# IntuitionMachines/volta

Measured on AMD Instinct MI355X. Metric: image-text pairs/sec, ctrl_vilbert_base pretrain step, higher is better.
Workload: dtype bf16

## Files before the change

### include/volta_hip.h

```cpp
#ifndef VOLTA_HIP_H
#define VOLTA_HIP_H
#include <stddef.h>
#include <stdint.h>

#ifdef __cplusplus
extern "C" {
#endif

typedef void* vk_stream_t;

int vk_version(void);
const char* vk_device_arch(void);
const char* vk_last_error(void);

typedef struct vk_dropout {
    const uint64_t* seed;
    uint32_t site;
    uint32_t threshold;
    float scale;
} vk_dropout;

int vk_set_seed(uint64_t* seed_dev, uint64_t seed, vk_stream_t s);

int vk_cast_f32_bf16(const float* src, void* dst, int64_t n, vk_stream_t s);
// ... 84 lines not shown

typedef struct vk_ln_bwd_args {
    const void* dy;
    const void* z;
    const float* mean;
    const float* rstd;
    const float* gamma;
    void* dz;
    void* dd;
    float* partial;
    float* dgamma;
    float* dbeta;
    const int32_t* dyn;
    int32_t M, H;
    int32_t split_row;
    int32_t post;
    float out_scale;
    int32_t accumulate;
    vk_dropout drop;
    vk_drop_rows seg[2];
} vk_ln_bwd_args;
int vk_ln_bwd_partial_rows(int M);
int vk_ln_bwd(const vk_ln_bwd_args* a, vk_stream_t s);
int vk_ln_bwd_pair(const vk_ln_bwd_args* a, const vk_ln_bwd_args* b, vk_stream_t s);
int vk_ln_bwd_finalize(const vk_ln_bwd_args* a, vk_stream_t s);

typedef struct vk_attn_args {
    const void* q[2];
    const void* k[2];
    const void* v[2];
    int32_t ld[2];
    int32_t L[2];
    const float* mask[2];
    void* ctx[2];
    int32_t ldo[2];
    float* lse[2];
    int32_t B, nh;
    int32_t gate[2][2];
    vk_dropout drop[2][2];
    float scale;
    int32_t dh;
    float* probs[2][2];
} vk_attn_args;
typedef struct vk_attn_bwd_args {
    const void* dctx[2];
    void* dq[2];
    void* dk[2];
    void* dv[2];
    int32_t ldg[2];
} vk_attn_bwd_args;
int vk_gated_attn_fwd(const vk_attn_args* a, vk_stream_t s);
int vk_gated_attn_bwd(const vk_attn_args* a, const vk_attn_bwd_args* b, vk_stream_t s);
size_t vk_gated_attn_lds_bytes(const vk_attn_args* a, int backward);

typedef struct vk_embed_args {
    const int64_t* ids;
    const int64_t* type_ids;
    const int64_t* pos_ids;
    const float* word;
    const float* pos;
    const float* type;
    const void* extra;
    void* z;
    int32_t M, T, H;
    int32_t V, P, n_types;
} vk_embed_args;
int vk_embed_sum_fwd(const vk_embed_args* a, vk_stream_t s);
typedef struct vk_embed_bwd_args {
    const void* dz;
    const int64_t* ids;
    const int64_t* type_ids;
    const int64_t* pos_ids;
    float* dword;
    float* dpos;
    float* dtype;
    int32_t M, T, H, n_types;
    int32_t V, P;
    void* work;
} vk_embed_bwd_args;
int64_t vk_embed_bwd_workspace_bytes(int M, int H, int V, int P, int has_pos);
int vk_embed_sum_bwd(const vk_embed_bwd_args* a, vk_stream_t s);

int vk_rows32(int M);
int vk_loc_linear_fwd(const float* loc, const float* W, const float* bias, void* out, int M, int H, int nloc, vk_stream_t s);
int vk_loc_linear_bwd(const void* dz, const float* loc, float* partial, float* dW, float* db, int M, int H, int nloc, vk_stream_t s);
int vk_add_dropout(const void* a, const void* b, void* y, int M, int H, float scale, vk_dropout drop, int backward, vk_stream_t s);
int vk_colsum_bf16(const void* src, float* partial, float* out, int M, int H, int accumulate, vk_stream_t s);
int vk_vlbert_prep_fwd(const float* loc, int nloc, const float* feat, const float* mask_emb, void* out, int32_t* zero_flag,
                       int M, int F, int dim, vk_dropout drop, vk_stream_t s);
int vk_vlbert_maskgrad(const void* dx, int ldx, int col0, const int32_t* zero_flag, float* partial, float* out, int M, int F,
                       vk_dropout drop, vk_stream_t s);
int vk_rowgroup_sum_bf16(const void* in, void* out, int B, int T, int H, vk_stream_t s);
int vk_relu_bwd_bf16(const void* dy, const void* y, void* out, int64_t n, vk_stream_t s);
int vk_copy_async(void* dst, const void* src, int64_t bytes, vk_stream_t s);
typedef struct vk_grad_seed_args {
    const float* src;
    int64_t stride_b, stride_l;
    void* dst;
    const void* y;
    int32_t B, L, H, row0, ld, ldy, accumulate, reserved_;
} vk_grad_seed_args;
int vk_grad_seed(const vk_grad_seed_args* a, vk_stream_t s);
#define VK_PAIR_MAX_SEGS 8
typedef struct vk_pair_gather_args {
    const void* src[VK_PAIR_MAX_SEGS];
    void* dst[VK_PAIR_MAX_SEGS];
// ... 539 lines not shown
```

### volta_amd/_lib.py

```python
import ctypes as C
import os

import torch

_HERE = os.path.dirname(os.path.abspath(__file__))
LIB_PATH = os.path.join(_HERE, "libvolta_hip_%s.so" % os.environ["VK_LIB"] if os.environ.get("VK_LIB") else "libvolta_hip.so")
GEMM_PERSISTENT, GEMM_ONE_TILE_PER_WG, GEMM_SOFT_START = 0x1000, 0x2000, 0x4000


class VoltaHipError(RuntimeError):
    pass


if not os.path.exists(LIB_PATH):
    raise ImportError(
        "volta_amd: %s not found. The HIP kernels are the product; there is no fallback path. "
        "Build with `make -C volta_amd/csrc` (hipcc --offload-arch=gfx950)." % LIB_PATH)

lib = C.CDLL(LIB_PATH)

c_p = C.c_void_p
i32 = C.c_int32
CHUNK_SKIP = 255

# ... 251 lines not shown
    _fields_ = [("fn", i32), ("p", c_p * 6), ("n", C.c_int64 * 6), ("f", C.c_float * 2), ("drop", Dropout)]


class Op(C.Structure):
    _fields_ = [("kind", i32), ("i0", i32), ("i1", i32), ("i2", i32), ("a", c_p), ("b", c_p), ("c", c_p)]


(OP_GEMM, OP_LN_FWD, OP_LN_BWD, OP_ATTN_FWD, OP_ATTN_BWD, OP_EMBED_FWD, OP_EMBED_BWD, OP_XENT_FWD, OP_XENT_BWD,
 OP_KL_FWD, OP_KL_BWD, OP_GENERIC, OP_SIDE_BEGIN, OP_SIDE_END, OP_WAIT_SIDE, OP_JOIN, OP_LN_FINALIZE, OP_GEMM_FP8, OP_GEMM_CHAIN) = range(1, 20)
(FN_CAST, FN_MEMSET, FN_LOC_FWD, FN_LOC_BWD, FN_ADD_DROPOUT, FN_COLSUM, FN_SELECT, FN_GATHER, FN_SCATTER_ADD,
 FN_LOSS_FINAL, FN_POOL_FWD, FN_POOL_BWD, FN_MASK_PREP, FN_MUL, FN_VLBERT_PREP, FN_VLBERT_MASKGRAD, FN_ROWGROUP_SUM,
 FN_RELU_BWD, FN_COPY, FN_SUM_SLABS, FN_SUM_SLABS_BF16, FN_SIDE_TAIL, FN_QUANT_ROWS, FN_CAST_FP8, FN_VIS_LOSS_FWD, FN_VIS_LOSS_BWD,
 FN_NCE_NEG, FN_TEXT_END_ROWS, FN_VLBERT_OBJ_IDS, FN_VLBERT_POSITIONS, FN_HOLD, FN_GATE, FN_BUMP, FN_GRAD_SEED, FN_LORA_FWD, FN_LORA_BWD,
 FN_LORA_PROJ_FWD, FN_LORA_PROJ_BWD, FN_LORA_FWD_DROP, FN_LORA_BWD_DROP, FN_LORA_PROJ_FWD_DROP, FN_LORA_PROJ_BWD_DROP) = range(1, 43)


class AttnArgs(C.Structure):
    _fields_ = [("q", c_p * 2), ("k", c_p * 2), ("v", c_p * 2), ("ld", i32 * 2), ("L", i32 * 2), ("mask", c_p * 2),
                ("ctx", c_p * 2), ("ldo", i32 * 2), ("lse", c_p * 2), ("B", i32), ("nh", i32), ("gate", (i32 * 2) * 2),
                ("drop", (Dropout * 2) * 2), ("scale", C.c_float), ("dh", i32), ("probs", (c_p * 2) * 2)]


class AttnBwdArgs(C.Structure):
    _fields_ = [("dctx", c_p * 2), ("dq", c_p * 2), ("dk", c_p * 2), ("dv", c_p * 2), ("ldg", i32 * 2)]


NT, NN, TN = 0, 1, 2
EPI_BF16, EPI_GELU, EPI_MULR, EPI_ADDR, EPI_F32, EPI_RELU, EPI_F32_ACC = range(7)


def _sig(name, restype, *argtypes):
    f = getattr(lib, name)
    f.restype = restype
    f.argtypes = list(argtypes)
    return f


_sig("vk_version", C.c_int)
_sig("vk_device_arch", C.c_char_p)
_sig("vk_last_error", C.c_char_p)
_sig("vk_set_seed", C.c_int, c_p, C.c_uint64, c_p)
_sig("vk_cast_f32_bf16", C.c_int, c_p, c_p, C.c_int64, c_p)
_sig("vk_gemm_grouped", C.c_int, C.c_int, C.c_int, C.POINTER(GemmProblem), C.c_int, c_p)
_sig("vk_gemm_fp8_grouped", C.c_int, C.c_int, C.POINTER(GemmFp8Problem), C.c_int, C.c_int, c_p)
_sig("vk_quant_rows_fp8", C.c_int, c_p, C.c_int, C.c_int64, c_p, C.c_int64, c_p, C.c_int, C.c_int, c_p, c_p)
_sig("vk_cast_bf16_fp8", C.c_int, c_p, c_p, C.c_int64, C.c_float, c_p)
_sig("vk_gemm_grouped_ex", C.c_int, C.c_int, C.c_int, C.POINTER(GemmProblem), C.c_int, C.c_int, c_p)
_sig("vk_gemm_geometry", C.c_int, C.c_int, C.c_int, C.POINTER(GemmProblem), C.c_int)
_sig("vk_gemm_chain", C.c_int, C.c_int, C.c_int, C.POINTER(GemmProblem), C.c_int, C.c_int, C.POINTER(GemmProblem), C.c_int, c_p)
_sig("vk_gemm_split_workspace_bytes", C.c_size_t, C.c_int, C.c_int, C.c_int, C.c_int, C.c_int, C.POINTER(C.c_int))
_sig("vk_gated_attn_fwd", C.c_int, C.POINTER(AttnArgs), c_p)
_sig("vk_gated_attn_bwd", C.c_int, C.POINTER(AttnArgs), C.POINTER(AttnBwdArgs), c_p)
_sig("vk_gated_attn_lds_bytes", C.c_size_t, C.POINTER(AttnArgs), C.c_int)
_sig("vk_ln_fwd", C.c_int, C.POINTER(LnArgs), c_p)
_sig("vk_ln_bwd_partial_rows", C.c_int, C.c_int)
_sig("vk_ln_bwd", C.c_int, C.POINTER(LnBwdArgs), c_p)
_sig("vk_embed_sum_fwd", C.c_int, C.POINTER(EmbedArgs), c_p)
_sig("vk_embed_sum_bwd", C.c_int, C.POINTER(EmbedBwdArgs), c_p)
_sig("vk_embed_bwd_workspace_bytes", C.c_int64, C.c_int, C.c_int, C.c_int, C.c_int, C.c_int)
_sig("vk_rows32", C.c_int, C.c_int)
_sig("vk_loc_linear_fwd", C.c_int, c_p, c_p, c_p, c_p, C.c_int, C.c_int, C.c_int, c_p)
_sig("vk_loc_linear_bwd", C.c_int, c_p, c_p, c_p, c_p, c_p, C.c_int, C.c_int, C.c_int, c_p)
_sig("vk_add_dropout", C.c_int, c_p, c_p, c_p, C.c_int, C.c_int, C.c_float, Dropout, C.c_int, c_p)
_sig("vk_colsum_bf16", C.c_int, c_p, c_p, c_p, C.c_int, C.c_int, C.c_int, c_p)
_sig("vk_vlbert_prep_fwd", C.c_int, c_p, C.c_int, c_p, c_p, c_p, c_p, C.c_int, C.c_int, C.c_int, Dropout, c_p)
_sig("vk_vlbert_maskgrad", C.c_int, c_p, C.c_int, C.c_int, c_p, c_p, c_p, C.c_int, C.c_int, Dropout, c_p)
_sig("vk_rowgroup_sum_bf16", C.c_int, c_p, c_p, C.c_int, C.c_int, C.c_int, c_p)
_sig("vk_relu_bwd_bf16", C.c_int, c_p, c_p, c_p, C.c_int64, c_p)
_sig("vk_copy_async", C.c_int, c_p, c_p, C.c_int64, c_p)
_sig("vk_select_rows", C.c_int, c_p, C.c_int, C.c_int, C.c_int, C.c_int, C.c_int, c_p, c_p, c_p, c_p)
_sig("vk_gather_rows", C.c_int, c_p, c_p, c_p, c_p, C.c_int, C.c_int, c_p)
_sig("vk_scatter_rows_add", C.c_int, c_p, c_p, c_p, c_p, C.c_int, C.c_int, c_p)
_sig("vk_xent_fwd", C.c_int, C.POINTER(XentArgs), c_p)
_sig("vk_xent_bwd", C.c_int, C.POINTER(XentArgs), c_p, C.c_int, c_p, c_p)
_sig("vk_kl_fwd", C.c_int, C.POINTER(KlArgs), c_p)
_sig("vk_kl_bwd", C.c_int, C.POINTER(KlArgs), c_p, C.c_int, c_p, c_p)
_sig("vk_loss_finalize", C.c_int, c_p, c_p, c_p, C.c_int, C.c_float, c_p, c_p)
_sig("vk_pool_mul_fwd", C.c_int, c_p, c_p, c_p, C.c_int, C.c_int, Dropout, c_p)
_sig("vk_pool_fuse_fwd", C.c_int, c_p, c_p, c_p, C.c_int, C.c_int, C.c_int, Dropout, c_p)
_sig("vk_pool_fuse_bwd", C.c_int, c_p, C.c_int, c_p, c_p, c_p, c_p, C.c_int, C.c_int, C.c_int, Dropout, c_p)
_sig("vk_text_end_rows", C.c_int, c_p, C.c_int, C.c_int, c_p, c_p, c_p)
_sig("vk_vlbert_obj_ids", C.c_int, c_p, c_p, C.c_int, C.c_int, c_p)
_sig("vk_lmdb_open", C.c_int, C.c_char_p, C.POINTER(c_p))
_sig("vk_lmdb_close", None, c_p)
_sig("vk_lmdb_entries", C.c_int64, c_p)
_sig("vk_lmdb_first", C.c_int, c_p)
_sig("vk_lmdb_next", C.c_int, c_p, C.POINTER(c_p), C.POINTER(C.c_size_t), C.POINTER(c_p), C.POINTER(C.c_size_t))
_sig("vk_lmdb_get", C.c_int, c_p, C.c_char_p, C.c_size_t, C.POINTER(c_p), C.POINTER(C.c_size_t))
_sig("vk_concap_record_decode", C.c_int, c_p, C.c_size_t, C.POINTER(ConcapRecord))
_sig("vk_concap_records_decode", C.c_int, C.POINTER(c_p), C.POINTER(C.c_size_t), C.POINTER(ConcapRecord), C.c_int, C.c_int, C.POINTER(C.c_int))
_sig("vk_wordpiece_open", C.c_int, C.c_char_p, C.c_int, C.POINTER(c_p))
_sig("vk_wordpiece_close", None, c_p)
_sig("vk_wordpiece_vocab_size", C.c_int, c_p)
_sig("vk_wordpiece_token_id", C.c_int, c_p, C.c_char_p)
_sig("vk_wordpiece_encode", C.c_int, c_p, C.c_char_p, C.c_size_t, c_p, C.c_int)
_sig("vk_wordpiece_encode_batch", C.c_int, c_p, C.POINTER(C.c_char_p), C.POINTER(C.c_size_t), C.c_int, c_p, C.c_int, c_p, C.c_int)
_sig("vk_b64_decode", C.c_int, C.c_char_p, C.c_size_t, c_p, C.c_size_t, C.POINTER(C.c_size_t))
_sig("vk_task_batch", C.c_int, C.POINTER(TaskBatchArgs), c_p)
_sig("vk_task_images_stage", C.c_int, C.POINTER(TaskImage), C.c_int, C.c_int, C.POINTER(C.c_int))
_sig("vk_task_batch_pool", C.c_int, C.POINTER(TaskPoolArgs), c_p)
_sig("vk_task_pool_means", C.c_int, C.POINTER(TaskPoolArgs), c_p, C.c_int, c_p)
_sig("vk_b64_decode_device", C.c_int, c_p, C.c_uint64, c_p, C.c_uint64, c_p, C.c_int, C.c_uint32, c_p, c_p)
_sig("vk_task_texts_pack", C.c_int, C.POINTER(TaskText), C.c_int, c_p, C.c_uint64, C.c_int)
_sig("vk_vlbert_positions", C.c_int, c_p, C.c_int, C.c_int, C.c_int, c_p, c_p, c_p)
_sig("vk_vis_loss_fwd", C.c_int, C.POINTER(VisLossArgs), c_p)
_sig("vk_vis_loss_bwd", C.c_int, C.POINTER(VisLossArgs), c_p, C.c_int, c_p, c_p)
# ... 12 lines not shown
_sig("vk_adamw_step_list", C.c_int, C.POINTER(AdamwArgs), c_p, C.c_int, C.c_int64, c_p)
_sig("vk_grad_sqnorm_list", C.c_int, c_p, C.c_int, C.c_int64, c_p, c_p, c_p)
_sig("vk_grad_sqnorm_list_work_floats", C.c_int)
_sig("vk_grad_seed", C.c_int, C.POINTER(GradSeedArgs), c_p)
_sig("vk_pair_gather", C.c_int, C.POINTER(PairGatherArgs), c_p)
_sig("vk_retrieval_ranks", C.c_int, C.POINTER(RetrievalRanksArgs), c_p)
_sig("vk_retrieval_ranks_shard_rows", C.c_int, C.POINTER(RetrievalRanksShardArgs), c_p)
_sig("vk_retrieval_ranks_shard_cols", C.c_int, C.POINTER(RetrievalRanksShardArgs), c_p)
_sig("vk_retrieval_ranks_finish", C.c_int, C.POINTER(RetrievalRanksShardArgs), c_p)
_sig("vk_image_means", C.c_int, C.POINTER(ImageMeansArgs), c_p)
_sig("vk_knn_pool_work_bytes", C.c_int64, C.c_int, C.c_int, C.c_int, C.c_int)
_sig("vk_knn_pool", C.c_int, C.POINTER(KnnPoolArgs), c_p)
_sig("vk_radam_step", C.c_int, C.POINTER(RadamArgs), c_p)
_sig("vk_radam_step_list", C.c_int, C.POINTER(RadamArgs), c_p, C.c_int, C.c_int64, c_p)
_sig("vk_lamb_work_bytes", C.c_int64, c_p, C.c_int, c_p, C.c_int, c_p, C.c_int)
_sig("vk_lamb_step", C.c_int, C.POINTER(LambArgs), c_p)
_sig("vk_lamb_step_timed", C.c_int, C.POINTER(LambArgs), c_p, C.POINTER(C.c_float))
_sig("vk_grad_sqnorm_chunks", C.c_int, c_p, C.c_int64, C.c_int64, c_p, c_p, c_p)
_sig("vk_grad_norm_from_chunks", C.c_int, c_p, C.c_int64, C.c_float, C.c_float, c_p, c_p)
_sig("vk_axpy_f32", C.c_int, c_p, c_p, C.c_float, C.c_int64, c_p)
_sig("vk_sum_slabs_f32", C.c_int, c_p, c_p, C.c_int64, C.c_int, C.c_int64, c_p)
_sig("vk_sum_slabs_bf16", C.c_int, c_p, c_p, C.c_int64, C.c_int, C.c_int64, c_p, C.c_int, c_p)
_sig("vk_memset_async", C.c_int, c_p, C.c_int, C.c_int64, c_p)
_sig("vk_hold_cus", C.c_int, C.c_int, C.c_int, C.c_int, c_p)
_sig("vk_gate_wait", C.c_int, c_p, c_p, C.c_int, c_p, c_p)
_sig("vk_bump_u64", C.c_int, c_p, c_p)
_sig("vk_store_u64", C.c_int, c_p, C.c_uint64, c_p)
_sig("vk_gate_value", C.c_int, c_p, C.c_uint64, C.c_int, c_p, c_p)
_sig("vk_comm_standin", C.c_int, c_p, c_p, C.c_int64, C.c_int, C.c_int, c_p, c_p)
_sig("vk_gemm_reserve_cus", C.c_int, C.c_int)
_sig("vk_side_tail", C.c_int, C.POINTER(TailJob), C.c_int, c_p)
_sig("vk_lora_fwd", C.c_int, C.POINTER(LoraProblem), C.c_int, c_p)
_sig("vk_lora_bwd", C.c_int, C.POINTER(LoraBwdProblem), C.c_int, c_p, c_p)
_sig("vk_lora_bwd_work_bytes", C.c_int64, C.POINTER(LoraBwdProblem), C.c_int)
_sig("vk_lora_proj_fwd", C.c_int, C.POINTER(LoraProjProblem), C.c_int, c_p)
_sig("vk_lora_proj_bwd", C.c_int, C.POINTER(LoraProjBwdProblem), C.c_int, c_p, c_p)
_sig("vk_lora_proj_bwd_work_bytes", C.c_int64, C.POINTER(LoraProjBwdProblem), C.c_int)
_sig("vk_lora_fwd_drop", C.c_int, C.POINTER(LoraProblem), C.POINTER(Dropout), C.c_int, c_p)
_sig("vk_lora_bwd_drop", C.c_int, C.POINTER(LoraBwdProblem), C.POINTER(Dropout), C.c_int, c_p, c_p)
_sig("vk_lora_proj_fwd_drop", C.c_int, C.POINTER(LoraProjProblem), C.POINTER(Dropout), C.c_int, c_p)
_sig("vk_lora_proj_bwd_drop", C.c_int, C.POINTER(LoraProjBwdProblem), C.POINTER(Dropout), C.c_int, c_p, c_p)
_sig("vk_run_ops", C.c_int, C.POINTER(Op), C.c_int, c_p)
_sig("vk_run_ops_timed", C.c_int, C.POINTER(Op), C.c_int, c_p, C.POINTER(C.c_float))
_sig("vk_ln_bwd_finalize", C.c_int, C.POINTER(LnBwdArgs), c_p)
_sig("vk_ln_fwd_pair", C.c_int, C.POINTER(LnArgs), C.POINTER(LnArgs), c_p)
_sig("vk_ln_bwd_pair", C.c_int, C.POINTER(LnBwdArgs), C.POINTER(LnBwdArgs), c_p)
_sig("vk_concap_batch", C.c_int, C.POINTER(ConcapArgs), c_p)
_sig("vk_side_join", C.c_int, c_p)
_sig("vk_side_join_from", C.c_int, c_p, c_p)
_sig("vk_side_enable", None, C.c_int)
_sig("vk_side_stream", c_p, c_p)

EXPORTS = ["vk_version", "vk_device_arch", "vk_last_error", "vk_set_seed", "vk_cast_f32_bf16", "vk_gemm_grouped", "vk_gemm_grouped_ex", "vk_gemm_geometry", "vk_gemm_chain", "vk_gemm_split_workspace_bytes", "vk_gemm_fp8_grouped", "vk_quant_rows_fp8", "vk_cast_bf16_fp8",
           "vk_ln_fwd", "vk_ln_fwd_pair", "vk_ln_bwd_partial_rows", "vk_ln_bwd", "vk_ln_bwd_pair", "vk_ln_bwd_finalize", "vk_gated_attn_fwd", "vk_gated_attn_bwd", "vk_gated_attn_lds_bytes",
           "vk_embed_sum_fwd", "vk_embed_sum_bwd", "vk_embed_bwd_workspace_bytes", "vk_rows32", "vk_loc_linear_fwd", "vk_loc_linear_bwd",
           "vk_add_dropout", "vk_colsum_bf16", "vk_vlbert_prep_fwd", "vk_vlbert_maskgrad", "vk_rowgroup_sum_bf16",
           "vk_relu_bwd_bf16", "vk_copy_async", "vk_select_rows", "vk_gather_rows", "vk_scatter_rows_add", "vk_xent_fwd",
           "vk_xent_bwd", "vk_kl_fwd", "vk_kl_bwd", "vk_loss_finalize", "vk_pool_mul_fwd", "vk_pool_mul_bwd",
           "vk_pool_fuse_fwd", "vk_pool_fuse_bwd", "vk_text_end_rows", "vk_vlbert_obj_ids", "vk_vlbert_positions", "vk_vis_loss_fwd", "vk_vis_loss_bwd", "vk_nce_negatives", "vk_task_loss_work_bytes", "vk_task_loss_fwd", "vk_task_loss_bwd",
           "vk_mask_prep", "vk_mul_bf16", "vk_grad_norm_workspace_floats", "vk_grad_norm_clip", "vk_grad_norm_clip_masked", "vk_grad_sqnorm_chunks", "vk_grad_norm_from_chunks", "vk_adamw_step", "vk_adamw_step_on", "vk_adamw_step_list", "vk_grad_sqnorm_list", "vk_grad_sqnorm_list_work_floats", "vk_grad_seed", "vk_pair_gather", "vk_radam_step", "vk_radam_step_list", "vk_lamb_work_bytes", "vk_lamb_step", "vk_lamb_step_timed",
           "vk_axpy_f32", "vk_sum_slabs_f32", "vk_sum_slabs_bf16", "vk_memset_async", "vk_hold_cus", "vk_gate_wait", "vk_bump_u64", "vk_store_u64", "vk_gate_value", "vk_comm_standin", "vk_gemm_reserve_cus", "vk_side_tail", "vk_run_ops", "vk_run_ops_timed", "vk_side_join", "vk_side_join_from", "vk_side_stream", "vk_side_enable", "vk_concap_batch",
           "vk_lmdb_open", "vk_lmdb_close", "vk_lmdb_entries", "vk_lmdb_first", "vk_lmdb_next", "vk_lmdb_get", "vk_concap_record_decode", "vk_concap_records_decode", "vk_b64_decode",
           "vk_wordpiece_open", "vk_wordpiece_close", "vk_wordpiece_vocab_size", "vk_wordpiece_token_id", "vk_wordpiece_encode", "vk_wordpiece_encode_batch",
           "vk_lora_fwd", "vk_lora_bwd", "vk_lora_bwd_work_bytes", "vk_lora_proj_fwd", "vk_lora_proj_bwd", "vk_lora_proj_bwd_work_bytes",
           "vk_lora_fwd_drop", "vk_lora_bwd_drop", "vk_lora_proj_fwd_drop", "vk_lora_proj_bwd_drop",
           "vk_task_batch", "vk_task_images_stage", "vk_task_batch_pool", "vk_task_pool_means", "vk_b64_decode_device", "vk_task_texts_pack", "vk_retrieval_ranks", "vk_retrieval_ranks_shard_rows", "vk_retrieval_ranks_shard_cols", "vk_retrieval_ranks_finish", "vk_image_means", "vk_knn_pool_work_bytes", "vk_knn_pool"]


def check(rc):
    if rc != 0:
        raise VoltaHipError(lib.vk_last_error().decode())


def stream_ptr():
    return C.c_void_p(torch.cuda.current_stream().cuda_stream)


def ptr(t):
    return C.c_void_p(t.data_ptr()) if t is not None else None
```

### volta_amd/csrc/attention.hip

```cpp
#include "common.h"
#include "../../include/volta_hip.h"
#include "util.h"

namespace vk {



template <int DHT>
__device__ __forceinline__ uint32_t img_off(int row, int col) {
    return (uint32_t)(row * (2 * DHT) + ((((col >> 4) ^ ((row >> 1) & 3)) << 5) | ((col & 15) << 1)));
}
template <int DHT>
__device__ __forceinline__ bf16x8 img_row_frag(uint32_t img, int row0, int ks, int lane) {
    const int row = row0 + (lane & 15);
    return *(const bf16x8 VK_LDS*)(uintptr_t)(img + img_off<DHT>(row, ks * 32 + (lane >> 4) * 8));
}
template <int DHT>
__device__ __forceinline__ bf16x8 img_tr_frag(uint32_t img, int rbase, int d0, int lane) {
    const int g = lane >> 4, q = (lane & 15) >> 2, p = lane & 3;
    const int r0 = rbase + 4 * g + q, r1 = r0 + 16;
    bf16x4 lo = lds_read_tr16(img + img_off<DHT>(r0, d0 + 4 * p));
    bf16x4 hi = lds_read_tr16(img + img_off<DHT>(r1, d0 + 4 * p));
    bf16x8 r;
    r[0] = lo[0]; r[1] = lo[1]; r[2] = lo[2]; r[3] = lo[3];
// ... 381 lines not shown
            f32x4 dq[DT];
#pragma unroll
            for (int dt = 0; dt < DT; ++dt) dq[dt] = f32x4{0.f, 0.f, 0.f, 0.f};
#define VK_QROLE(MK)                                                                                       \
            if (a.gate[mq][MK]) {                                                                          \
                const int Lk = a.L[MK];                                                                    \
                const vk_dropout dc = a.drop[mq][MK];                                                      \
                const bool don = dc.threshold != 0;                                                        \
                const uint64_t seed = don ? *dc.seed : 0;                                                  \
                _Pragma("unroll") for (int pp = 0; pp < NKT[MK] / 2; ++pp) {                               \
                    if (pp * 32 < Lk) {                                                                    \
                        f32x4 ds[2];                                                                       \
                        _Pragma("unroll") for (int hh = 0; hh < 2; ++hh) {                                 \
                            const int kt = pp * 2 + hh;                                                    \
                            ds[hh] = f32x4{0.f, 0.f, 0.f, 0.f};                                            \
                            if (kt * 16 >= Lk) continue;                   \
                            f32x4 s = {0.f, 0.f, 0.f, 0.f}, dp = {0.f, 0.f, 0.f, 0.f};                     \
                            _Pragma("unroll") for (int ks = 0; ks < KS; ++ks) {                            \
                                s = __builtin_amdgcn_mfma_f32_16x16x32_bf16(img_row_frag<DHT>(kimg[MK], kt * 16, ks, lane), qf[ks], s, 0, 0, 0); \
                                dp = __builtin_amdgcn_mfma_f32_16x16x32_bf16(img_row_frag<DHT>(vimg[MK], kt * 16, ks, lane), gf[ks], dp, 0, 0, 0); \
                            }                                                                              \
                            u32x4 w = {~0u, ~0u, ~0u, ~0u};                                                \
                            if (don) w = philox4((uint32_t)(kt * 4 + g), drow, dc.site, 0u, (uint32_t)seed, (uint32_t)(seed >> 32)); \
                            _Pragma("unroll") for (int r = 0; r < 4; ++r) {                                \
                                const int key = kt * 16 + 4 * g + r;                                       \
                                float v = 0.f;                                                             \
                                if (key < Lk && qvalid) {                                                  \
                                    const float p = __expf(s[r] * a.scale + mask_s[rbase[MK] + key] - lse);      \
                                    const float keep = (w[r] >= dc.threshold) ? dc.scale : 0.f;            \
                                    v = p * (dp[r] * keep - delta);                                        \
                                }                                                                          \
                                ds[hh][r] = v;                                                             \
                            }                                                                              \
                        }                                                                                  \
                        const bf16x8 sb = pack_pair(ds[0], ds[1]);                                         \
                        _Pragma("unroll") for (int dt = 0; dt < DT; ++dt)                                  \
                            dq[dt] = __builtin_amdgcn_mfma_f32_16x16x32_bf16(img_tr_frag<DHT>(kimg[MK], pp * 32, dt * 16, lane), sb, dq[dt], 0, 0, 0); \
                    }                                                                                      \
                }                                                                                          \
            }
            VK_QROLE(0)
            VK_QROLE(1)
#undef VK_QROLE
            if (qvalid) {
                const size_t off = ((size_t)b * Lq + qi) * a.ldg[mq] + h * DHT + 4 * g;
#pragma unroll
                for (int dt = 0; dt < DT; ++dt)
                    *(u32x2*)(a.dq[mq] + off + dt * 16) = u32x2{pack2bf(dq[dt][0] * a.scale, dq[dt][1] * a.scale), pack2bf(dq[dt][2] * a.scale, dq[dt][3] * a.scale)};
            }
        }
    }
}

#ifdef VK_STUDY
#define VK_ATTN_TUNABLE static int
#else
#define VK_ATTN_TUNABLE static constexpr int
#endif

static int fill(AttnK& k, const vk_attn_args* a, const vk_attn_bwd_args* bw) {
    for (int m = 0; m < 2; ++m) {
        k.q[m] = (const uint16_t*)a->q[m]; k.k[m] = (const uint16_t*)a->k[m]; k.v[m] = (const uint16_t*)a->v[m];
        k.ld[m] = a->ld[m]; k.L[m] = a->L[m]; k.mask[m] = a->mask[m];
        k.ctx[m] = (uint16_t*)a->ctx[m]; k.ldo[m] = a->ldo[m]; k.lse[m] = a->lse[m];
        for (int n = 0; n < 2; ++n) { k.gate[m][n] = a->gate[m][n]; k.drop[m][n] = a->drop[m][n]; }
        k.dctx[m] = bw ? (const uint16_t*)bw->dctx[m] : nullptr;
        k.dq[m] = bw ? (uint16_t*)bw->dq[m] : nullptr; k.dk[m] = bw ? (uint16_t*)bw->dk[m] : nullptr;
        k.dv[m] = bw ? (uint16_t*)bw->dv[m] : nullptr; k.ldg[m] = bw ? bw->ldg[m] : 0;
    }
    k.B = a->B; k.nh = a->nh; k.scale = a->scale;
    for (int m = 0; m < 2; ++m) {
        const bool qa = a->gate[m][0] || a->gate[m][1], ka = a->gate[0][m] || a->gate[1][m];
        if (!qa && !ka) continue;
        if (a->L[m] <= 0) return set_error("vk_gated_attn: modality %d is gated on but has length %d", m, a->L[m]);
        if (a->L[m] > (m == 0 ? 64 : 128)) return set_error("vk_gated_attn: lengths (%d, %d) exceed the (64, 128) tile budget", a->L[0], a->L[1]);
        if ((a->ld[m] & 7) || (a->ldo[m] & 7)) return set_error("vk_gated_attn: row strides must be multiples of 8");
        if (ka && (!a->k[m] || !a->v[m] || !a->mask[m])) return set_error("vk_gated_attn: K/V/mask of modality %d missing", m);
        if (qa && (!a->q[m] || !a->ctx[m] || !a->lse[m])) return set_error("vk_gated_attn: Q/ctx/lse of modality %d missing", m);
        if (bw && qa && (!bw->dctx[m] || !bw->dq[m])) return set_error("vk_gated_attn_bwd: dctx/dq of modality %d missing", m);
        if (bw && ka && (!bw->dk[m] || !bw->dv[m])) return set_error("vk_gated_attn_bwd: dk/dv of modality %d missing", m);
    }
    return 0;
}

VK_ATTN_TUNABLE g_attn_fwd_waves = 4;
VK_ATTN_TUNABLE g_attn_fwd_occ = 4;
template <int TP, int RP, int DHT>
static int launch_fwd(const AttnK& k, int nq_tiles, hipStream_t s) {
    const int lds = 3 * (TP + RP) * 2 * DHT + (TP + RP) * 4 + 16;
    int waves = nq_tiles < 4 ? 4 : (nq_tiles > 8 ? 8 : nq_tiles);
    if (g_attn_fwd_waves >= 4 && g_attn_fwd_waves < waves && 4 * lds <= 160 * 1024) waves = g_attn_fwd_waves;
    if (DHT == 64 && g_attn_fwd_occ == 5) {
        hipLaunchKernelGGL((attn_fwd_kernel<TP, RP, 5, DHT>), dim3(k.B * k.nh), dim3(64 * waves), lds, s, k);
    } else {
        auto kern = attn_fwd_kernel<TP, RP, (DHT == 64 ? 4 : 3), DHT>;
        static const hipError_t attr = hipFuncSetAttribute((const void*)kern, hipFuncAttributeMaxDynamicSharedMemorySize, lds); (void)attr;
        hipLaunchKernelGGL(kern, dim3(k.B * k.nh), dim3(64 * waves), lds, s, k);
    }
    return check_launch("vk_gated_attn_fwd");
}
VK_ATTN_TUNABLE g_attn_bwd_waves = 4;
VK_ATTN_TUNABLE g_attn_bwd_occ = 3;

template <int TP, int RP, int DHT>
static int launch_bwd(const AttnK& k, int ntasks, hipStream_t s) {
    const int lds = 4 * (TP + RP) * 2 * DHT + 3 * (TP + RP) * 4 + 16;
    if (DHT == 64 && g_attn_bwd_occ == 3 && 3 * lds <= 160 * 1024) {
        auto kern = attn_bwd_kernel<TP, RP, 3, DHT>;
        static const hipError_t attr = hipFuncSetAttribute((const void*)kern, hipFuncAttributeMaxDynamicSharedMemorySize, lds); (void)attr;
        int waves = g_attn_bwd_waves < 4 ? 4 : (ntasks > g_attn_bwd_waves ? g_attn_bwd_waves : (ntasks < 4 ? 4 : ntasks));
        hipLaunchKernelGGL(kern, dim3(k.B * k.nh), dim3(64 * waves), lds, s, k);
    } else {
        auto kern = attn_bwd_kernel<TP, RP, 2, DHT>;
        static const hipError_t attr = hipFuncSetAttribute((const void*)kern, hipFuncAttributeMaxDynamicSharedMemorySize, lds); (void)attr;
        int waves = g_attn_bwd_waves < 4 ? 4 : (ntasks > g_attn_bwd_waves ? g_attn_bwd_waves : (ntasks < 4 ? 4 : ntasks));
        if (2 * lds > 160 * 1024) waves = ntasks >= 8 ? 8 : (ntasks < 4 ? 4 : ntasks);
        hipLaunchKernelGGL(kern, dim3(k.B * k.nh), dim3(64 * waves), lds, s, k);
    }
    return check_launch("vk_gated_attn_bwd");
}

static bool bwd_fits(int TP, int RP, int dht) { return 4 * (TP + RP) * 2 * dht + 3 * (TP + RP) * 4 + 16 <= 160 * 1024; }

}

namespace vk { int attn_generic(const vk_attn_args* a, const vk_attn_bwd_args* bw, vk_stream_t stream); }

#ifdef VK_STUDY
static int g_attn_force_generic = 0;
extern "C" void vk_attn_set_force_generic(int v) { g_attn_force_generic = v; }
#else
static constexpr int g_attn_force_generic = 0;
#endif
static bool attn_mfma_ok(const vk_attn_args* a) {
    if (a->probs[0][0] || a->probs[0][1] || a->probs[1][0] || a->probs[1][1]) return false;
    for (int m = 0; m < 2; ++m) {
        const bool on = a->gate[m][0] || a->gate[m][1] || a->gate[0][m] || a->gate[1][m];
        if (on && a->L[m] > (m == 0 ? 64 : 128)) return false;
    }
    if (a->dh == 0 || a->dh == 64) return true;
    if (a->dh != 128 || g_attn_force_generic) return false;
    const int TP = a->L[0] > 32 ? 64 : 32, RP = a->L[1] > 64 ? 128 : 64;
    return vk::bwd_fits(TP, RP, 128);
}

namespace vk { size_t attn_generic_lds(const vk_attn_args* a, bool bwd); }

extern "C" size_t vk_gated_attn_lds_bytes(const vk_attn_args* a, int backward) {
    if (!a || attn_mfma_ok(a)) return 0;
    return vk::attn_generic_lds(a, backward != 0);
}

extern "C" int vk_gated_attn_fwd(const vk_attn_args* a, vk_stream_t stream) {
    using namespace vk;
    if (!attn_mfma_ok(a)) return attn_generic(a, nullptr, stream);
    AttnK k;
    if (int rc = fill(k, a, nullptr)) return rc;
    if (a->B <= 0) return 0;
    int nq = 0;
    for (int m = 0; m < 2; ++m) if (a->gate[m][0] || a->gate[m][1]) nq += (a->L[m] + 15) / 16;
    hipStream_t s = (hipStream_t)stream;
    const bool bigT = a->L[0] > 32, bigR = a->L[1] > 64;
    if (a->dh == 128) {
        if (!bigT && !bigR) return launch_fwd<32, 64, 128>(k, nq, s);
        return launch_fwd<64, 64, 128>(k, nq, s);
    }
    if (!bigT && !bigR) return launch_fwd<32, 64, 64>(k, nq, s);
    if (bigT && !bigR) return launch_fwd<64, 64, 64>(k, nq, s);
    if (!bigT && bigR) return launch_fwd<32, 128, 64>(k, nq, s);
    return launch_fwd<64, 128, 64>(k, nq, s);
}

extern "C" int vk_gated_attn_bwd(const vk_attn_args* a, const vk_attn_bwd_args* bw, vk_stream_t stream) {
    using namespace vk;
    if (!attn_mfma_ok(a)) return attn_generic(a, bw, stream);
    AttnK k;
    if (int rc = fill(k, a, bw)) return rc;
    if (a->B <= 0) return 0;
    int nt = 0;
    for (int m = 0; m < 2; ++m) {
        if (a->gate[m][0] || a->gate[m][1]) nt += (a->L[m] + 15) / 16;
        if (a->gate[0][m] || a->gate[1][m]) nt += (a->L[m] + 15) / 16;
    }
    hipStream_t s = (hipStream_t)stream;
    const bool bigT = a->L[0] > 32, bigR = a->L[1] > 64;
    if (a->dh == 128) {
        if (!bigT && !bigR) return launch_bwd<32, 64, 128>(k, nt, s);
        return launch_bwd<64, 64, 128>(k, nt, s);
    }
    if (!bigT && !bigR) return launch_bwd<32, 64, 64>(k, nt, s);
    if (bigT && !bigR) return launch_bwd<64, 64, 64>(k, nt, s);
    if (!bigT && bigR) return launch_bwd<32, 128, 64>(k, nt, s);
    return launch_bwd<64, 128, 64>(k, nt, s);
}
#ifdef VK_STUDY
extern "C" void vk_attn_set_bwd_occupancy(int v) { vk::g_attn_bwd_occ = v; }
extern "C" void vk_attn_set_bwd_waves(int v) { vk::g_attn_bwd_waves = v; }
extern "C" void vk_attn_set_fwd_waves(int v) { vk::g_attn_fwd_waves = v; }
extern "C" void vk_attn_set_fwd_occupancy(int v) { vk::g_attn_fwd_occ = v; }
#endif
```

Before: 15550.

## Add one-wave-per-head attention kernels for short text-only sequences

Adds specialized forward and backward gated-attention kernels for the text-only self-attention case with at most 32 rows and head dim 64. Each wave handles one (batch, head) pair, several waves share a block, and synchronization uses wave-level LDS fences instead of block barriers. This targets the launch and occupancy overhead of the general tiled kernels when sequences are short. The path is on by default with a runtime switch to disable it. It adds a second code path that must match the original dropout and mask semantics.

```diff
diff --git a/include/volta_hip.h b/include/volta_hip.h
--- a/include/volta_hip.h
+++ b/include/volta_hip.h
@@ -160,6 +160,7 @@
 int vk_gated_attn_fwd(const vk_attn_args* a, vk_stream_t s);
 int vk_gated_attn_bwd(const vk_attn_args* a, const vk_attn_bwd_args* b, vk_stream_t s);
 size_t vk_gated_attn_lds_bytes(const vk_attn_args* a, int backward);
+void vk_attn_short_path(int on);
 
 typedef struct vk_embed_args {
     const int64_t* ids;
diff --git a/volta_amd/_lib.py b/volta_amd/_lib.py
--- a/volta_amd/_lib.py
+++ b/volta_amd/_lib.py
@@ -327,6 +327,7 @@
 _sig("vk_gated_attn_fwd", C.c_int, C.POINTER(AttnArgs), c_p)
 _sig("vk_gated_attn_bwd", C.c_int, C.POINTER(AttnArgs), C.POINTER(AttnBwdArgs), c_p)
 _sig("vk_gated_attn_lds_bytes", C.c_size_t, C.POINTER(AttnArgs), C.c_int)
+_sig("vk_attn_short_path", None, C.c_int)
 _sig("vk_ln_fwd", C.c_int, C.POINTER(LnArgs), c_p)
 _sig("vk_ln_bwd_partial_rows", C.c_int, C.c_int)
 _sig("vk_ln_bwd", C.c_int, C.POINTER(LnBwdArgs), c_p)
@@ -445,7 +446,7 @@
 _sig("vk_side_stream", c_p, c_p)
 
 EXPORTS = ["vk_version", "vk_device_arch", "vk_last_error", "vk_set_seed", "vk_cast_f32_bf16", "vk_gemm_grouped", "vk_gemm_grouped_ex", "vk_gemm_geometry", "vk_gemm_chain", "vk_gemm_split_workspace_bytes", "vk_gemm_fp8_grouped", "vk_quant_rows_fp8", "vk_cast_bf16_fp8",
-           "vk_ln_fwd", "vk_ln_fwd_pair", "vk_ln_bwd_partial_rows", "vk_ln_bwd", "vk_ln_bwd_pair", "vk_ln_bwd_finalize", "vk_gated_attn_fwd", "vk_gated_attn_bwd", "vk_gated_attn_lds_bytes",
+           "vk_ln_fwd", "vk_ln_fwd_pair", "vk_ln_bwd_partial_rows", "vk_ln_bwd", "vk_ln_bwd_pair", "vk_ln_bwd_finalize", "vk_gated_attn_fwd", "vk_gated_attn_bwd", "vk_gated_attn_lds_bytes", "vk_attn_short_path",
            "vk_embed_sum_fwd", "vk_embed_sum_bwd", "vk_embed_bwd_workspace_bytes", "vk_rows32", "vk_loc_linear_fwd", "vk_loc_linear_bwd",
            "vk_add_dropout", "vk_colsum_bf16", "vk_vlbert_prep_fwd", "vk_vlbert_maskgrad", "vk_rowgroup_sum_bf16",
            "vk_relu_bwd_bf16", "vk_copy_async", "vk_select_rows", "vk_gather_rows", "vk_scatter_rows_add", "vk_xent_fwd",
diff --git a/volta_amd/csrc/attention.hip b/volta_amd/csrc/attention.hip
--- a/volta_amd/csrc/attention.hip
+++ b/volta_amd/csrc/attention.hip
@@ -457,6 +457,322 @@
     }
 }
 
+constexpr int SHORT_ROWS = 32;
+#ifndef VK_ATTN_SHORT_WAVES
+#define VK_ATTN_SHORT_WAVES 4
+#endif
+constexpr int SHORT_WAVES = VK_ATTN_SHORT_WAVES;
+static_assert(SHORT_WAVES >= 1 && SHORT_WAVES <= 5, "the short backward asks for SHORT_WAVES x 12672 bytes of LDS without raising the limit");
+
+__device__ __forceinline__ void wave_lds_sync() {
+    __builtin_amdgcn_fence(__ATOMIC_RELEASE, "wavefront");
+    __builtin_amdgcn_wave_barrier();
+    __builtin_amdgcn_fence(__ATOMIC_ACQUIRE, "wavefront");
+}
+template <int DHT>
+__device__ __forceinline__ bf16x8 glb_row_frag(const uint16_t* base, int ld, int L, int row0, int ks, int lane) {
+    const int row = row0 + (lane & 15);
+    u32x4 r = *(const u32x4*)(base + (size_t)(row < L ? row : 0) * ld + ks * 32 + (lane >> 4) * 8);
+    if (row >= L) r = u32x4{0u, 0u, 0u, 0u};
+    return __builtin_bit_cast(bf16x8, r);
+}
+template <int DHT>
+__device__ __forceinline__ void wave_load(u32x4 (&r)[DHT / 16], const uint16_t* base, int ld, int L, int lane) {
+    constexpr int CH = DHT / 8;
+#pragma unroll
+    for (int i = 0; i < DHT / 16; ++i) {
+        const int idx = i * 64 + lane, row = idx / CH, ch = idx % CH;
+        r[i] = *(const u32x4*)(base + (size_t)(row < L ? row : 0) * ld + ch * 8);
+        if (row >= L) r[i] = u32x4{0u, 0u, 0u, 0u};
+    }
+}
+template <int DHT>
+__device__ __forceinline__ void wave_store(uint32_t img, const u32x4 (&r)[DHT / 16], int lane) {
+    constexpr int CH = DHT / 8;
+#pragma unroll
+    for (int i = 0; i < DHT / 16; ++i) {
+        const int idx = i * 64 + lane, row = idx / CH, ch = idx % CH;
+        *(u32x4 VK_LDS*)(uintptr_t)(img + img_off<DHT>(row, ch * 8)) = r[i];
+    }
+}
+template <int DHT>
+__device__ __forceinline__ void wave_delta(const u32x4 (&rg)[DHT / 16], const u32x4 (&ro)[DHT / 16], float VK_LDS* del_s, int lane) {
+    constexpr int CH = DHT / 8;
+#pragma unroll
+    for (int i = 0; i < DHT / 16; ++i) {
+        const int idx = i * 64 + lane, row = idx / CH, ch = idx % CH;
+        float part = 0.f;
+#pragma unroll
+        for (int k = 0; k < 4; ++k)
+            part += bf2f(rg[i][k] & 0xFFFF) * bf2f(ro[i][k] & 0xFFFF) + bf2f(rg[i][k] >> 16) * bf2f(ro[i][k] >> 16);
+        part += __shfl_xor(part, 1, 64);
+        part += __shfl_xor(part, 2, 64);
+        part += __shfl_xor(part, 4, 64);
+        if (CH > 8) part += __shfl_xor(part, 8, 64);
+        if (ch == 0) del_s[row] = part;
+    }
+}
+
+template <int DHT> struct ShortLds {
+    static constexpr int FWD = SHORT_ROWS * 2 * DHT + SHORT_ROWS * 4;
+    static constexpr int BWD = 3 * SHORT_ROWS * 2 * DHT + 3 * SHORT_ROWS * 4;
+};
+
+template <int DHT>
+__global__ __launch_bounds__(64 * SHORT_WAVES) void attn_fwd_short_kernel(const AttnK a) {
+    extern __shared__ __attribute__((aligned(16))) char smem[];
+    constexpr int NKT = SHORT_ROWS / 16, NQT = SHORT_ROWS / 16;
+    constexpr int KS = DHT / 32, DT = DHT / 16;
+    const int lane = threadIdx.x & 63;
+    const int wave = __builtin_amdgcn_readfirstlane((int)(threadIdx.x >> 6));
+    const int u = blockIdx.x * SHORT_WAVES + wave;
+    if (u >= a.B * a.nh) return;
+    const uint32_t vimg = (uint32_t)(uintptr_t)(VK_LDS char*)smem + wave * ShortLds<DHT>::FWD;
+    float VK_LDS* const mask_s = (float VK_LDS*)(uintptr_t)(vimg + SHORT_ROWS * 2 * DHT);
+    const int b = u / a.nh, h = u - b * a.nh;
+    const int g = lane >> 4, lq = lane & 15;
+    const int L = a.L[0], ld = a.ld[0];
+    const size_t roff = ((size_t)b * L) * ld + h * DHT;
+
+    u32x4 rv[DHT / 16];
+    bf16x8 kf[NKT][KS], qf[NQT][KS];
+    wave_load<DHT>(rv, a.v[0] + roff, ld, L, lane);
+#pragma unroll
+    for (int t = 0; t < NKT; ++t)
+#pragma unroll
+        for (int ks = 0; ks < KS; ++ks) {
+            kf[t][ks] = glb_row_frag<DHT>(a.k[0] + roff, ld, L, t * 16, ks, lane);
+            qf[t][ks] = glb_row_frag<DHT>(a.q[0] + roff, ld, L, t * 16, ks, lane);
+        }
+    const int ml = lane & (SHORT_ROWS - 1);
+    float mk = a.mask[0][(size_t)b * L + (ml < L ? ml : 0)];
+    if (ml >= L) mk = 0.f;
+    wave_store<DHT>(vimg, rv, lane);
+    mask_s[ml] = mk;
+    wave_lds_sync();
+
+    const vk_dropout dc = a.drop[0][0];
+    const bool don = dc.threshold != 0;
+    const uint64_t seed = don ? *dc.seed : 0;
+#pragma unroll
+    for (int qt = 0; qt < NQT; ++qt) {
+        if (qt * 16 >= L) break;
+        const int qi = qt * 16 + lq;
+        const bool qvalid = qi < L;
+        const int qc = qvalid ? qi : L - 1;
+        f32x4 s0[NKT];
+        float mx = -INFINITY;
+#pragma unroll
+        for (int kt = 0; kt < NKT; ++kt) {
+            s0[kt] = f32x4{-INFINITY, -INFINITY, -INFINITY, -INFINITY};
+            if (kt * 16 < L) {
+                f32x4 acc = {0.f, 0.f, 0.f, 0.f};
+#pragma unroll
+                for (int ks = 0; ks < KS; ++ks)
+                    acc = __builtin_amdgcn_mfma_f32_16x16x32_bf16(kf[kt][ks], qf[qt][ks], acc, 0, 0, 0);
+                const f32x4 mk4 = *(const f32x4 VK_LDS*)(mask_s + kt * 16 + 4 * g);
+#pragma unroll
+                for (int r = 0; r < 4; ++r) {
+                    const int key = kt * 16 + 4 * g + r;
+                    if (key < L) {
+                        s0[kt][r] = acc[r] * a.scale + mk4[r];
+                        mx = fmaxf(mx, s0[kt][r]);
+                    }
+                }
+            }
+        }
+        mx = group_max(mx);
+        float sum = 0.f;
+#pragma unroll
+        for (int kt = 0; kt < NKT; ++kt)
+#pragma unroll
+            for (int r = 0; r < 4; ++r) { s0[kt][r] = __expf(s0[kt][r] - mx); sum += s0[kt][r]; }
+        sum = group_sum(sum);
+        const float inv = 1.0f / sum;
+        if (qvalid && g == 0) a.lse[0][((size_t)b * a.nh + h) * L + qi] = mx + __logf(sum);
+        const uint32_t drow = (uint32_t)(((size_t)b * a.nh + h) * L + qc);
+
+        f32x4 o[DT];
+#pragma unroll
+        for (int dt = 0; dt < DT; ++dt) o[dt] = f32x4{0.f, 0.f, 0.f, 0.f};
+#pragma unroll
+        for (int kt = 0; kt < NKT; ++kt) {
+            u32x4 w = {~0u, ~0u, ~0u, ~0u};
+            if (don && kt * 16 < L)
+                w = philox4((uint32_t)(kt * 4 + g), drow, dc.site, 0u, (uint32_t)seed, (uint32_t)(seed >> 32));
+#pragma unroll
+            for (int r = 0; r < 4; ++r)
+                s0[kt][r] = (w[r] >= dc.threshold) ? s0[kt][r] * inv * dc.scale : 0.f;
+        }
+        const bf16x8 pb = pack_pair(s0[0], s0[1]);
+#pragma unroll
+        for (int dt = 0; dt < DT; ++dt)
+            o[dt] = __builtin_amdgcn_mfma_f32_16x16x32_bf16(img_tr_frag<DHT>(vimg, 0, dt * 16, lane), pb, o[dt], 0, 0, 0);
+        if (qvalid) {
+            uint16_t* orow = a.ctx[0] + ((size_t)b * L + qi) * a.ldo[0] + h * DHT + 4 * g;
+#pragma unroll
+            for (int dt = 0; dt < DT; ++dt)
+                *(u32x2*)(orow + dt * 16) = u32x2{pack2bf(o[dt][0], o[dt][1]), pack2bf(o[dt][2], o[dt][3])};
+        }
+    }
+}
+
+template <int DHT>
+__global__ __launch_bounds__(64 * SHORT_WAVES) void attn_bwd_short_kernel(const AttnK a) {
+    extern __shared__ __attribute__((aligned(16))) char smem[];
+    constexpr int NT = SHORT_ROWS / 16;
+    constexpr int RB = 2 * DHT, KS = DHT / 32, DT = DHT / 16;
+    const int lane = threadIdx.x & 63;
+    const int wave = __builtin_amdgcn_readfirstlane((int)(threadIdx.x >> 6));
+    const int u = blockIdx.x * SHORT_WAVES + wave;
+    if (u >= a.B * a.nh) return;
+    const uint32_t qimg = (uint32_t)(uintptr_t)(VK_LDS char*)smem + wave * ShortLds<DHT>::BWD;
+    const uint32_t gimg = qimg + SHORT_ROWS * RB, kimg = gimg + SHORT_ROWS * RB;
+    float VK_LDS* const lse_s = (float VK_LDS*)(uintptr_t)(kimg + SHORT_ROWS * RB);
+    float VK_LDS* const del_s = lse_s + SHORT_ROWS;
+    float VK_LDS* const mask_s = del_s + SHORT_ROWS;
+    const int b = u / a.nh, h = u - b * a.nh;
+    const int g = lane >> 4, lq = lane & 15;
+    const int L = a.L[0];
+    const size_t roff = ((size_t)b * L) * a.ld[0] + h * DHT, ooff = ((size_t)b * L) * a.ldo[0] + h * DHT;
+
+    u32x4 rq[DHT / 16], rg[DHT / 16], ro[DHT / 16], rk[DHT / 16];
+    bf16x8 vfr[NT][KS];
+    wave_load<DHT>(rk, a.k[0] + roff, a.ld[0], L, lane);
+    wave_load<DHT>(rq, a.q[0] + roff, a.ld[0], L, lane);
+    wave_load<DHT>(rg, a.dctx[0] + ooff, a.ldo[0], L, lane);
+    wave_load<DHT>(ro, a.ctx[0] + ooff, a.ldo[0], L, lane);
+#pragma unroll
+    for (int t = 0; t < NT; ++t)
+#pragma unroll
+        for (int ks = 0; ks < KS; ++ks) vfr[t][ks] = glb_row_frag<DHT>(a.v[0] + roff, a.ld[0], L, t * 16, ks, lane);
+    const int ml = lane & (SHORT_ROWS - 1);
+    float mkv = a.mask[0][(size_t)b * L + (ml < L ? ml : 0)];
+    float lsev = a.lse[0][((size_t)b * a.nh + h) * L + (ml < L ? ml : 0)];
+    if (ml >= L) { mkv = 0.f; lsev = 0.f; }
+    __builtin_amdgcn_sched_barrier(0);
+    wave_store<DHT>(kimg, rk, lane);
+    wave_store<DHT>(qimg, rq, lane);
+    wave_store<DHT>(gimg, rg, lane);
+    wave_delta<DHT>(rg, ro, del_s, lane);
+    mask_s[ml] = mkv; lse_s[ml] = lsev;
+    wave_lds_sync();
+
+    const vk_dropout dc = a.drop[0][0];
+    const bool don = dc.threshold != 0;
+    const uint64_t seed = don ? *dc.seed : 0;
+#pragma unroll
+    for (int kt = 0; kt < NT; ++kt) {
+        if (kt * 16 >= L) break;
+        const int key = kt * 16 + lq;
+        const bool kvalid = key < L;
+        const float kmask = kvalid ? mask_s[key] : 0.f;
+        bf16x8 kf[KS];
+#pragma unroll
+        for (int ks = 0; ks < KS; ++ks) kf[ks] = img_row_frag<DHT>(kimg, kt * 16, ks, lane);
+        f32x4 dk[DT], dv[DT];
+#pragma unroll
+        for (int dt = 0; dt < DT; ++dt) { dk[dt] = f32x4{0.f, 0.f, 0.f, 0.f}; dv[dt] = f32x4{0.f, 0.f, 0.f, 0.f}; }
+        f32x4 pd[2], ds[2];
+#pragma unroll
+        for (int hh = 0; hh < 2; ++hh) {
+            const int qt = hh;
+            pd[hh] = f32x4{0.f, 0.f, 0.f, 0.f}; ds[hh] = f32x4{0.f, 0.f, 0.f, 0.f};
+            if (qt * 16 >= L) continue;
+            f32x4 s = {0.f, 0.f, 0.f, 0.f}, dp = {0.f, 0.f, 0.f, 0.f};
+#pragma unroll
+            for (int ks = 0; ks < KS; ++ks) {
+                s = __builtin_amdgcn_mfma_f32_16x16x32_bf16(img_row_frag<DHT>(qimg, qt * 16, ks, lane), kf[ks], s, 0, 0, 0);
+                dp = __builtin_amdgcn_mfma_f32_16x16x32_bf16(img_row_frag<DHT>(gimg, qt * 16, ks, lane), vfr[kt][ks], dp, 0, 0, 0);
+            }
+            const f32x4 lse4 = *(const f32x4 VK_LDS*)(lse_s + qt * 16 + 4 * g), del4 = *(const f32x4 VK_LDS*)(del_s + qt * 16 + 4 * g);
+            uint32_t wr[4] = {~0u, ~0u, ~0u, ~0u};
+            if (don) {
+                const uint32_t drow_t = (uint32_t)(((size_t)b * a.nh + h) * L + (qt * 16 + 4 * g + (lq & 3)));
+                const u32x4 wq = philox4((uint32_t)(key >> 2), drow_t, dc.site, 0u, (uint32_t)seed, (uint32_t)(seed >> 32));
+                wr[0] = quad_word<0>(wq, lq & 3); wr[1] = quad_word<1>(wq, lq & 3);
+                wr[2] = quad_word<2>(wq, lq & 3); wr[3] = quad_word<3>(wq, lq & 3);
+            }
+#pragma unroll
+            for (int r = 0; r < 4; ++r) {
+                const int qi = qt * 16 + 4 * g + r;
+                float p = 0.f, keep = 1.f;
+                if (qi < L && kvalid) {
+                    p = __expf(s[r] * a.scale + kmask - lse4[r]);
+                    if (don) keep = (wr[r] >= dc.threshold) ? dc.scale : 0.f;
+                }
+                pd[hh][r] = p * keep;
+                ds[hh][r] = p * (dp[r] * keep - del4[r]);
+            }
+        }
+        const bf16x8 pb = pack_pair(pd[0], pd[1]), sb = pack_pair(ds[0], ds[1]);
+#pragma unroll
+        for (int dt = 0; dt < DT; ++dt) {
+            dv[dt] = __builtin_amdgcn_mfma_f32_16x16x32_bf16(img_tr_frag<DHT>(gimg, 0, dt * 16, lane), pb, dv[dt], 0, 0, 0);
+            dk[dt] = __builtin_amdgcn_mfma_f32_16x16x32_bf16(img_tr_frag<DHT>(qimg, 0, dt * 16, lane), sb, dk[dt], 0, 0, 0);
+        }
+        if (kvalid) {
+            const size_t off = ((size_t)b * L + key) * a.ldg[0] + h * DHT + 4 * g;
+#pragma unroll
+            for (int dt = 0; dt < DT; ++dt) {
+                *(u32x2*)(a.dk[0] + off + dt * 16) = u32x2{pack2bf(dk[dt][0] * a.scale, dk[dt][1] * a.scale), pack2bf(dk[dt][2] * a.scale, dk[dt][3] * a.scale)};
+                *(u32x2*)(a.dv[0] + off + dt * 16) = u32x2{pack2bf(dv[dt][0], dv[dt][1]), pack2bf(dv[dt][2], dv[dt][3])};
+            }
+        }
+    }
+#pragma unroll
+    for (int qt = 0; qt < NT; ++qt) {
+        if (qt * 16 >= L) break;
+        const int qi = qt * 16 + lq;
+        const bool qvalid = qi < L;
+        bf16x8 qf[KS], gf[KS];
+#pragma unroll
+        for (int ks = 0; ks < KS; ++ks) { qf[ks] = img_row_frag<DHT>(qimg, qt * 16, ks, lane); gf[ks] = img_row_frag<DHT>(gimg, qt * 16, ks, lane); }
+        const float lse = lse_s[qt * 16 + lq], delta = del_s[qt * 16 + lq];
+        const uint32_t drow = (uint32_t)(((size_t)b * a.nh + h) * L + (qvalid ? qi : 0));
+        f32x4 dq[DT];
+#pragma unroll
+        for (int dt = 0; dt < DT; ++dt) dq[dt] = f32x4{0.f, 0.f, 0.f, 0.f};
+        f32x4 ds[2];
+#pragma unroll
+        for (int hh = 0; hh < 2; ++hh) {
+            const int kt = hh;
+            ds[hh] = f32x4{0.f, 0.f, 0.f, 0.f};
+            if (kt * 16 >= L) continue;
+            f32x4 s = {0.f, 0.f, 0.f, 0.f}, dp = {0.f, 0.f, 0.f, 0.f};
+#pragma unroll
+            for (int ks = 0; ks < KS; ++ks) {
+                s = __builtin_amdgcn_mfma_f32_16x16x32_bf16(img_row_frag<DHT>(kimg, kt * 16, ks, lane), qf[ks], s, 0, 0, 0);
+                dp = __builtin_amdgcn_mfma_f32_16x16x32_bf16(vfr[kt][ks], gf[ks], dp, 0, 0, 0);
+            }
+            const f32x4 mk4 = *(const f32x4 VK_LDS*)(mask_s + kt * 16 + 4 * g);
+            u32x4 w = {~0u, ~0u, ~0u, ~0u};
+            if (don) w = philox4((uint32_t)(kt * 4 + g), drow, dc.site, 0u, (uint32_t)seed, (uint32_t)(seed >> 32));
+#pragma unroll
+            for (int r = 0; r < 4; ++r) {
+                const int key = kt * 16 + 4 * g + r;
+                float v = 0.f;
+                if (key < L && qvalid) {
+                    const float p = __expf(s[r] * a.scale + mk4[r] - lse);
+                    const float keep = (w[r] >= dc.threshold) ? dc.scale : 0.f;
+                    v = p * (dp[r] * keep - delta);
+                }
+                ds[hh][r] = v;
+            }
+        }
+        const bf16x8 sb = pack_pair(ds[0], ds[1]);
+#pragma unroll
+        for (int dt = 0; dt < DT; ++dt)
+            dq[dt] = __builtin_amdgcn_mfma_f32_16x16x32_bf16(img_tr_frag<DHT>(kimg, 0, dt * 16, lane), sb, dq[dt], 0, 0, 0);
+        if (qvalid) {
+            const size_t off = ((size_t)b * L + qi) * a.ldg[0] + h * DHT + 4 * g;
+#pragma unroll
+            for (int dt = 0; dt < DT; ++dt)
+                *(u32x2*)(a.dq[0] + off + dt * 16) = u32x2{pack2bf(dq[dt][0] * a.scale, dq[dt][1] * a.scale), pack2bf(dq[dt][2] * a.scale, dq[dt][3] * a.scale)};
+        }
+    }
+}
+
 #ifdef VK_STUDY
 #define VK_ATTN_TUNABLE static int
 #else
@@ -525,6 +841,17 @@
     return check_launch("vk_gated_attn_bwd");
 }
 
+static int launch_fwd_short(const AttnK& k, hipStream_t s) {
+    const int units = k.B * k.nh;
+    hipLaunchKernelGGL((attn_fwd_short_kernel<64>), dim3((units + SHORT_WAVES - 1) / SHORT_WAVES), dim3(64 * SHORT_WAVES), SHORT_WAVES * ShortLds<64>::FWD, s, k);
+    return check_launch("vk_gated_attn_fwd (short rows)");
+}
+static int launch_bwd_short(const AttnK& k, hipStream_t s) {
+    const int units = k.B * k.nh;
+    hipLaunchKernelGGL((attn_bwd_short_kernel<64>), dim3((units + SHORT_WAVES - 1) / SHORT_WAVES), dim3(64 * SHORT_WAVES), SHORT_WAVES * ShortLds<64>::BWD, s, k);
+    return check_launch("vk_gated_attn_bwd (short rows)");
+}
+
 static bool bwd_fits(int TP, int RP, int dht) { return 4 * (TP + RP) * 2 * dht + 3 * (TP + RP) * 4 + 16 <= 160 * 1024; }
 
 }
@@ -551,6 +878,12 @@
 
 namespace vk { size_t attn_generic_lds(const vk_attn_args* a, bool bwd); }
 
+static int g_attn_short_path = 1;
+extern "C" void vk_attn_short_path(int on) { g_attn_short_path = on != 0; }
+static bool attn_short_ok(const vk_attn_args* a) {
+    return g_attn_short_path && a->gate[0][0] && !a->gate[0][1] && !a->gate[1][0] && !a->gate[1][1] && a->L[0] <= vk::SHORT_ROWS && (a->dh == 0 || a->dh == 64);
+}
+
 extern "C" size_t vk_gated_attn_lds_bytes(const vk_attn_args* a, int backward) {
     if (!a || attn_mfma_ok(a)) return 0;
     return vk::attn_generic_lds(a, backward != 0);
@@ -562,6 +895,7 @@
     AttnK k;
     if (int rc = fill(k, a, nullptr)) return rc;
     if (a->B <= 0) return 0;
+    if (attn_short_ok(a)) return launch_fwd_short(k, (hipStream_t)stream);
     int nq = 0;
     for (int m = 0; m < 2; ++m) if (a->gate[m][0] || a->gate[m][1]) nq += (a->L[m] + 15) / 16;
     hipStream_t s = (hipStream_t)stream;
@@ -582,6 +916,7 @@
     AttnK k;
     if (int rc = fill(k, a, bw)) return rc;
     if (a->B <= 0) return 0;
+    if (attn_short_ok(a)) return launch_bwd_short(k, (hipStream_t)stream);
     int nt = 0;
     for (int m = 0; m < 2; ++m) {
         if (a->gate[m][0] || a->gate[m][1]) nt += (a->L[m] + 15) / 16;
```

New measurement: 15630, median of 6. Within noise of the previous version (+0.5%).
